# zhengchen1999/DOVE

Measured on AMD Instinct MI355X. Metric: SR frames/s (33x720x1280 4x one-step, whole job), higher is better.
Workload: dtype bf16; 1 GPU; synthetic 33x720x1280 HR clip (LR 180x320, 4x), one-step t=399, CogVideoX1.5-5B VAE + 42-layer DiT random-init, 1 clip per GPU (BASELINE configs[1]); weight_sums=True, vae_streams=2, variant=headline (bf16)

## Files before the change

### dove_amd/csrc/igemm.hip

```cpp
#include "igemm_args.h"


template <int BN, int BK>
struct FastCfg {
  static constexpr int BM = 128;
  static constexpr int CPR = BK / 8;
  static constexpr int CPR_LOG = (BK == 64) ? 3 : 2;
  static constexpr int RPG = 256 / CPR;
  static constexpr int NA = BM / RPG;
  static constexpr int B_SLOTS = BN * CPR;
  static constexpr int NB = (B_SLOTS + 255) / 256;
  static constexpr int A_BYTES = BM * BK * 2, B_BYTES = BN * BK * 2, STAGE = A_BYTES + B_BYTES;
  static constexpr int WN = (BN >= 128) ? 2 : 1, WM = 4 / WN;
  static constexpr int PT = (BM / WM) / 32, CT = (BN / WN) / 32;
  static constexpr int KK = BK / 16;
};

template <int BN, int BK>
__global__ __launch_bounds__(256) void igemm_fast_kernel(const IgemmArgs a) {
  using Cf = FastCfg<BN, BK>;
  constexpr int NA = Cf::NA, NB = Cf::NB, PT = Cf::PT, CT = Cf::CT, KK = Cf::KK, STAGE = Cf::STAGE, A_BYTES = Cf::A_BYTES;
  extern __shared__ __attribute__((aligned(16))) char smem[];
  const int tid = threadIdx.x, lane = tid & 63;
  const int wave = __builtin_amdgcn_readfirstlane(tid >> 6);
// ... 546 lines not shown
      mfma16(32 + 2 * g, wh[(2 * g) >> 3], xs[SP][(2 * g) & 7]);
      mfma16(32 + 2 * g + 1, wh[(2 * g + 1) >> 3], xs[SP][(2 * g + 1) & 7]);
      if (g < 8) {
        int ad;
        if (tap < NT - 1) ad = a16_addr(std::integral_constant<int, (tap + 1) % NT>{}, Par{}, g);
        else if (kSub) ad = a16_addr_next0(NPar{}, g);
        else ad = a16_addr(I0{}, NPar{}, g);
        xs[SP ^ 1][g] = *(const bf16x8*)(smem + ad);
      } else if (g < 12) {
        wl[g - 8] = *(const bf16x8*)(smem + b16_addr(SlotNxt{}, g - 8));
      }
      __builtin_amdgcn_sched_barrier(0);
    }
  };
  auto group = [&](auto parc) {
    step(std::integral_constant<int, 0>{}, parc); step(std::integral_constant<int, 1>{}, parc);
    step(std::integral_constant<int, 2>{}, parc); step(std::integral_constant<int, 3>{}, parc);
    if (!kSub) {
      step(std::integral_constant<int, (kSub ? 0 : 4)>{}, parc); step(std::integral_constant<int, (kSub ? 0 : 5)>{}, parc);
      step(std::integral_constant<int, (kSub ? 0 : 6)>{}, parc); step(std::integral_constant<int, (kSub ? 0 : 7)>{}, parc);
      step(std::integral_constant<int, (kSub ? 0 : 8)>{}, parc);
    }
  };

  const int e_px = lane >> 3, e_ch = lane & 7;
  for (int tile = (int)blockIdx.x; tile < ntiles; tile += G) {
    const H4Tile c = h4_decode<kPart>(a, kc, tile);
    f32x4 bias_r[2][2];
#pragma unroll
    for (int h = 0; h < 2; ++h) {
      const int cbh = c.n0 + h * 64 + e_ch * 8;
      bias_r[h][0] = bias_r[h][1] = f32x4{0.f, 0.f, 0.f, 0.f};
      if (a.bias) { bias_r[h][0] = *(const f32x4*)(a.bias + cbh); bias_r[h][1] = *(const f32x4*)(a.bias + cbh + 4); }
    }
#pragma unroll
    for (int k = 0; k < 64; ++k) acc16[k] = f32x4{0.f, 0.f, 0.f, 0.f};

    const int ng_tile = h4_split_ndt(a, __builtin_amdgcn_readfirstlane(h4_split(a, c.t))) * kc.kcn;
    int next_base0 = 0;
    if (kSub) {
      sub_bases(c.ph, abaseT);
      int nb4[4];
      sub_bases(h4_decode(a, kc, tile + G).ph, nb4);
      next_base0 = nb4[0];
    }
#pragma unroll
    for (int idx = 0; idx < 8; ++idx) xs[0][idx] = *(const bf16x8*)(smem + a16_addr(I0{}, I0{}, idx));
#pragma unroll
    for (int ib = 0; ib < 4; ++ib) wl[ib] = *(const bf16x8*)(smem + b16_addr(I0{}, ib));
    for (int g = 0; g < ng_tile; g += 2) {
      if (kSub) abaseN0 = abaseT[0];
      group(I0{});
      __builtin_amdgcn_sched_barrier(0);
      h4_advance<kUp, kPart>(st, a, kc);
      publish(st);
      __builtin_amdgcn_sched_barrier(0);
      if (kSub) abaseN0 = (g + 2 >= ng_tile) ? next_base0 : abaseT[0];
      group(I1{});
      __builtin_amdgcn_sched_barrier(0);
      h4_advance<kUp, kPart>(st, a, kc);
      publish(st);
      __builtin_amdgcn_sched_barrier(0);
    }

    __builtin_amdgcn_s_barrier();
    {
      constexpr int EROW = 272;
      char* const eslice = smem + A_BYTES + wave * 12288;
      unsigned o_off[4], r_off[4];
#pragma unroll
      for (int it = 0; it < 4; ++it) {
        const int px = it * 8 + e_px;
        if (kPart == 1) {
          const int col = px & 15, row = px >> 4;
          const bool okw = c.ow0 + col < a.w_lim;
          o_off[it] = okw ? (unsigned)(((row * a.W_out + col) * (int)a.ldo + e_ch * 8) * 2) : 0x80000000u;
          r_off[it] = okw ? (unsigned)(((row * a.W_out + col) * (int)a.ldr + e_ch * 8) * 2) : 0x80000000u;
          continue;
        }
        const bool okw = kSub ? c.ow0 + px < a.W_in : c.ow0 + px < a.w_lim;
        o_off[it] = okw ? (unsigned)(((kSub ? 2 * px : px) * (int)a.ldo + e_ch * 8) * 2) : 0x80000000u;
        r_off[it] = okw ? (unsigned)((px * (int)a.ldr + e_ch * 8) * 2) : 0x80000000u;
      }
      auto emit = [&](auto has_resid, auto has_gn) {
        constexpr bool kRes = decltype(has_resid)::value;
        constexpr bool kGn = decltype(has_gn)::value;
        typedef __attribute__((ext_vector_type(2))) float f32x2;
        f32x2 gs[2][2], gq[2][2];
#pragma unroll
        for (int h = 0; h < 2; ++h)
#pragma unroll
          for (int q2 = 0; q2 < 2; ++q2) { gs[h][q2] = f32x2{0.f, 0.f}; gq[h][q2] = f32x2{0.f, 0.f}; }
        auto wr = [&](int p, int h) {
#pragma unroll
          for (int ib = 0; ib < 4; ++ib)
#pragma unroll
            for (int j = 0; j < 2; ++j) *(f32x4*)(eslice + (16 * j + l15) * EROW + (ib * 16 + 4 * q4) * 4) = acc16[(h * 4 + ib) * 8 + 2 * p + j];
          (void)hi; (void)l31;
        };
        auto gn_flush = [&](int half) {
          const int cpg_log = a.cpg_log;
          const int gty = (c.oh0 >> 4) + (kPart == 1 ? wave >> 1 : 0), gtx = c.ow0 >> 5;
          const int slot = kPart == 1 ? 2 * (wave & 1) + half : wave;
          const long long tix = ((long long)c.t * a.tiles_h + gty) * a.tiles_w + gtx;
          const long long row = ((kSub ? tix * 4 + c.ph : tix) << 2) + slot;
          float* dst = a.gn_partial + row * 64;
          const bool own = kPart != 1 || (gty < a.tiles_h && gty * 16 < a.h_lim);
#pragma unroll
          for (int h = 0; h < 2; ++h) {
            float sv[2], qv[2];
#pragma unroll
            for (int q2 = 0; q2 < 2; ++q2) {
              sv[q2] = gs[h][q2][0] + gs[h][q2][1];
              qv[q2] = gq[h][q2][0] + gq[h][q2][1];
#pragma unroll
              for (int m = 8; m < 64; m <<= 1) { sv[q2] += __shfl_xor(sv[q2], m); qv[q2] += __shfl_xor(qv[q2], m); }
              gs[h][q2] = f32x2{0.f, 0.f}; gq[h][q2] = f32x2{0.f, 0.f};
            }
            const int ch0 = c.n0 + h * 64 + e_ch * 8;
            if (cpg_log == 2) {
              if (e_px == 0 && own) {
                dst[(ch0 >> 2) * 2] = sv[0]; dst[(ch0 >> 2) * 2 + 1] = qv[0];
                dst[((ch0 >> 2) + 1) * 2] = sv[1]; dst[((ch0 >> 2) + 1) * 2 + 1] = qv[1];
              }
            } else {
              float s8 = sv[0] + sv[1], q8 = qv[0] + qv[1];
              if (cpg_log == 4) { s8 += __shfl_xor(s8, 1); q8 += __shfl_xor(q8, 1); }
              const bool writer = e_px == 0 && (cpg_log == 3 || (e_ch & 1) == 0);
              if (writer && own) { dst[(ch0 >> cpg_log) * 2] = s8; dst[(ch0 >> cpg_log) * 2 + 1] = q8; }
            }
          }
        };
        wr(0, 0);
#pragma unroll
        for (int p = 0; p < 4; ++p) {
          const int oh = c.oh0 + RPW * wave + (kPart == 1 ? 2 * p : p);
          const long long pix0 = kSub ? ((long long)c.t * a.H_out + 2 * oh + (c.ph >> 1)) * a.W_out + 2 * c.ow0 + (c.ph & 1)
                                      : ((long long)c.t * a.H_out + oh) * a.W_out + c.ow0;
          const bool okh = kSub ? oh < a.H_in : oh < a.h_lim;
          const int span_px = kSub ? 2 * halo8::TW : (kPart == 1 ? a.W_out + 16 : halo8::TW);
          const auto srd_o = __builtin_amdgcn_make_buffer_rsrc((void*)(a.out + pix0 * a.ldo + c.n0), (short)0,
                                                               okh ? (int)(span_px * a.ldo * 2) : 0, 0x00020000);
          const auto srd_r = __builtin_amdgcn_make_buffer_rsrc((void*)(kRes ? a.resid + pix0 * a.ldr + c.n0 : a.out), (short)0,
                                                               (kRes && okh) ? (int)((kPart == 1 ? a.W_out + 16 : halo8::TW) * a.ldr * 2) : 0, 0x00020000);
          unsigned oo[4], ro[4];
          const bool ok1 = oh + 1 < a.h_lim;
#pragma unroll
          for (int it = 0; it < 4; ++it) {
            if (kPart == 1) { oo[it] = (it >= 2 && !ok1) ? 0x80000000u : o_off[it]; ro[it] = (it >= 2 && !ok1) ? 0x80000000u : r_off[it]; }
            else { oo[it] = o_off[it]; ro[it] = r_off[it]; }
          }
#pragma unroll
          for (int h = 0; h < 2; ++h) {
            u32x4 rr[4];
            if (kRes) {
#pragma unroll
              for (int it = 0; it < 4; ++it) rr[it] = __builtin_amdgcn_raw_buffer_load_b128(srd_r, (int)ro[it], h * 128, 0);
            }
            asm volatile("s_waitcnt lgkmcnt(0)" ::: "memory");
            f32x4 lo[4], hi4[4];
#pragma unroll
            for (int it = 0; it < 4; ++it) {
              lo[it] = *(const f32x4*)(eslice + (it * 8 + e_px) * EROW + e_ch * 32);
              hi4[it] = *(const f32x4*)(eslice + (it * 8 + e_px) * EROW + e_ch * 32 + 16);
            }
            asm volatile("s_waitcnt lgkmcnt(0)" ::: "memory");
            if (p < 3 || h < 1) wr(h ? p + 1 : p, h ^ 1);
#pragma unroll
            for (int it = 0; it < 4; ++it) {
              f32x4 x0 = lo[it] + bias_r[h][0], x1 = hi4[it] + bias_r[h][1];
              if (kRes) {
                const u32x4 r = rr[it];
                x0 += f32x4{__uint_as_float(r[0] << 16), __uint_as_float(r[0] & 0xffff0000u), __uint_as_float(r[1] << 16),
                            __uint_as_float(r[1] & 0xffff0000u)};
                x1 += f32x4{__uint_as_float(r[2] << 16), __uint_as_float(r[2] & 0xffff0000u), __uint_as_float(r[3] << 16),
                            __uint_as_float(r[3] & 0xffff0000u)};
              }
              const u32x4 v = {pack_bf2(x0[0], x0[1]), pack_bf2(x0[2], x0[3]), pack_bf2(x1[0], x1[1]), pack_bf2(x1[2], x1[3])};
              if (kGn) {
                const bool valid = okh && oo[it] != 0x80000000u;
#pragma unroll
                for (int e = 0; e < 4; ++e) {
                  const uint32_t w = valid ? v[e] : 0u;
                  const f32x2 f = {__uint_as_float(w << 16), __uint_as_float(w & 0xffff0000u)};
                  gs[h][e >> 1] += f;
                  gq[h][e >> 1] += f * f;
                }
              }
              __builtin_amdgcn_raw_buffer_store_b128(v, srd_o, (int)oo[it], h * 128, 0);
              __builtin_amdgcn_sched_barrier(0);
              asm volatile("s_nop 3" ::: "memory");
              __builtin_amdgcn_sched_barrier(0);
            }
          }
          if (kGn && kPart == 1 && p == 1) gn_flush(0);
        }
        if (kGn) gn_flush(kPart == 1 ? 1 : 0);
      };
      if (a.gn_partial) {
        if (a.resid) emit(std::true_type{}, std::true_type{});
        else emit(std::false_type{}, std::true_type{});
      } else {
        if (a.resid) emit(std::true_type{}, std::false_type{});
        else emit(std::false_type{}, std::false_type{});
      }
    }
    asm volatile("s_waitcnt vmcnt(0)" ::: "memory");
  }
}

namespace gemm8p {
constexpr int ROWB = 128;
constexpr int OPB = 256 * ROWB;
constexpr int XB = 0, WB = 2 * OPB;
constexpr int EPI = 4 * OPB;
constexpr int LDS_BYTES = EPI + 8 * 4096;
}
template <bool kAct, bool kGate>
__global__ __launch_bounds__(512, 2) void gemm8p_kernel(const IgemmArgs a, long long M) {
  using gemm4x::BM;
  using namespace gemm8p;
  extern __shared__ __attribute__((aligned(16))) char smem[];
  const int tid = threadIdx.x, lane = tid & 63;
  const int wave = __builtin_amdgcn_readfirstlane(tid >> 6);
  __builtin_assume(wave >= 0 && wave < 8);
  const int hi = lane >> 5, l31 = lane & 31;
  const int q4 = lane >> 4, l15 = lane & 15;
  const int grp = wave >> 2, wc = wave & 3;

  G4Const kc;
  kc.K = a.Cin;
  kc.M = M;
  kc.tiles_n = a.tiles_n;
  kc.ntiles = (int)((M + BM - 1) / BM) * a.tiles_n;
  kc.G = (int)gridDim.x;
  kc.nk4 = a.Cin / 128;
  const int ntiles = kc.ntiles, G = kc.G, nk4 = kc.nk4;

  unsigned voff[4];
#pragma unroll
  for (int jj = 0; jj < 4; ++jj) {
    const int row = (wave * 4 + jj) * 8 + (lane >> 3);
    const int c = (lane & 7) ^ ((row >> 1) & 7);
    voff[jj] = (unsigned)((row * a.Cin + c * 8) * 2);
  }
  G4State st;
  const bf16_t *ca_base = a.x, *cw_base = a.w, *na_base = a.x, *nw_base = a.w;
  int ca_nrec = 0, cw_nrec = 0, c_soff = 0, na_nrec = 0, nw_nrec = 0, n_soff = 0;
  auto publish = [&](const G4State& q) {
    ca_base = na_base; cw_base = nw_base; ca_nrec = na_nrec; cw_nrec = nw_nrec; c_soff = n_soff;
    na_base = q.a_base; nw_base = q.w_base; na_nrec = q.a_nrec; nw_nrec = q.w_nrec; n_soff = q.soff;
  };
  auto stage = [&](auto bufc, const bf16_t* ab, int anrec, const bf16_t* wb, int wnrec, int soff) {
    constexpr int buf = decltype(bufc)::value;
    const auto srd_a = __builtin_amdgcn_make_buffer_rsrc((void*)ab, (short)0, anrec, 0x00020000);
    const auto srd_w = __builtin_amdgcn_make_buffer_rsrc((void*)wb, (short)0, wnrec, 0x00020000);
#pragma unroll
    for (int jj = 0; jj < 4; ++jj)
      __builtin_amdgcn_raw_ptr_buffer_load_lds(srd_a, (lds_ptr_t)(smem + XB + buf * OPB + wave * 4096 + jj * 1024), 16, voff[jj], soff, 0, 0);
#pragma unroll
    for (int jj = 0; jj < 4; ++jj)
      __builtin_amdgcn_raw_ptr_buffer_load_lds(srd_w, (lds_ptr_t)(smem + WB + buf * OPB + wave * 4096 + jj * 1024), 16, voff[jj], soff, 0, 0);
  };

  int aoff[2][2], boff[2][2];
  {
    const int ra = grp * 128 + l31, rb = wc * 64 + l31;
#pragma unroll
    for (int h = 0; h < 2; ++h)
#pragma unroll
      for (int kk = 0; kk < 2; ++kk) {
        const int ch = h * 4 + kk * 2 + hi;
        aoff[h][kk] = XB + ra * ROWB + ((ch ^ ((ra >> 1) & 7)) << 4);
        boff[h][kk] = WB + rb * ROWB + ((ch ^ ((rb >> 1) & 7)) << 4);
        asm volatile("" : "+v"(aoff[h][kk]), "+v"(boff[h][kk]));
// ... 265 lines not shown
                          d->t_in == d->t_out && d->h_in == d->h_out && d->w_in == d->w_out && d->cout_pad % 128 == 0 && M >= 4096 &&
                          (long long)512 * d->cin * 2 < (1ll << 31);
  const bool pointwise = d->kt == 1 && d->kh == 1 && d->kw == 1 && d->stride == 1 && d->up == 0 && d->tmode == 0 && d->t_in == d->t_out &&
                         d->h_in == d->h_out && d->w_in == d->w_out;
  if (pointwise && d->cin == 32 && d->act == 0 && !d->resid && !d->gate && d->cout_store >= 128) return K_SMALLK;
  if (plain_gemm) {
    if (d->cout_pad % 256 == 0 && d->cout_store % 256 == 0 && d->cin % 128 == 0 && d->cin >= 256 && (long long)256 * d->cin * 2 < (1ll << 31) &&
        d->ldo < (1 << 20) && d->ldr < (1 << 20) && (d->act == 0 || d->act == 1))
      return K_GEMM8P;
  }
  const bool conv3 = d->kh == 3 && d->kw == 3 && d->stride == 1 && d->pad_h == 1 && d->pad_w == 1 && d->act == 0 && !d->gate &&
                     d->cout_pad % 128 == 0 && frame_fits;
  if (conv3) {
    const bool same = d->up == 0 && d->tmode == 0 && d->h_out == d->h_in && d->w_out == d->w_in && d->w_out >= 16 && d->h_out >= 16;
    const bool ups = d->up == 1 && d->kt == 1 && d->h_out == 2 * d->h_in && d->w_out == 2 * d->w_in && d->h_out >= 16 && d->w_out >= 32;
    const bool h4 = d->cout_store % 128 == 0 && d->cin % 64 == 0 && d->ldo < (1 << 20) && (!d->resid || d->ldr < (1 << 20));
    if (same && h4) return K_HALO4X;
    if (ups && h4 && d->w_sub && d->h_in >= 16 && d->w_in >= 32) return K_HALO4X_SUB;
    if (ups && h4) return K_HALO4X_UP;
  }
  const int BN = (d->cout_pad % 128 == 0) ? 128 : ((d->cout_pad % 64 == 0) ? 64 : 32);
  const bool fits = frame_fits && (long long)BN * d->cin * 2 < (1ll << 31);
  return (d->up == 0 && fits) ? K_IGEMM_FAST : K_IGEMM;
}

static bool desc_size_ok(const dove_conv_desc* d, const char* who) {
  if (d && d->struct_size == sizeof(dove_conv_desc) && d->reserved == 0) return true;
  if (d) dove_set_error("%s: dove_conv_desc.struct_size is %u, this library (ABI %d) expects %zu - the caller's binding was written "
                        "against another include/dove_hip.h", who, d->struct_size, DOVE_ABI_VERSION, sizeof(dove_conv_desc));
  else dove_set_error("%s: null descriptor", who);
  return false;
}
extern "C" const char* dove_conv_kernel_name(const dove_conv_desc* d) { return desc_size_ok(d, "conv_kernel_name") ? kKernelNames[select_kernel(d)] : ""; }

template <int BN, int BK>
static int launch_igemm_fast(const IgemmArgs& a, unsigned grid, hipStream_t s) {
  constexpr int lds = 2 * (128 * BK * 2 + BN * BK * 2);
  static PerDeviceOnce attr_set;
  if (auto once_ = attr_set.guard()) (void)hipFuncSetAttribute((const void*)igemm_fast_kernel<BN, BK>, hipFuncAttributeMaxDynamicSharedMemorySize, lds);
  hipLaunchKernelGGL((igemm_fast_kernel<BN, BK>), dim3(grid), dim3(256), lds, s, a);
  DOVE_CHECK_LAUNCH("dove_conv_igemm_bf16");
  return DOVE_OK;
}

static int cu_count() {
  static std::atomic<int> cus[DOVE_MAX_DEVICES] = {};
  int dev = 0;
  (void)hipGetDevice(&dev);
  int n = (dev >= 0 && dev < DOVE_MAX_DEVICES) ? cus[dev].load(std::memory_order_relaxed) : 0;
  if (!n) {
    n = 256;
    (void)hipDeviceGetAttribute(&n, hipDeviceAttributeMultiprocessorCount, dev);
    if (dev >= 0 && dev < DOVE_MAX_DEVICES) cus[dev].store(n, std::memory_order_relaxed);
  }
  return n;
}

extern "C" long long dove_conv_gn_partial_rows(const dove_conv_desc* d) {
  if (!desc_size_ok(d, "conv_gn_partial_rows")) return 0;
  const ConvKernel k = select_kernel(d);
  if (k != K_HALO4X && k != K_HALO4X_UP && k != K_HALO4X_SUB) return 0;
  if (d->cout_store != 128 && d->cout_store != 256 && d->cout_store != 512) return 0;
  if (d->cout_store != d->cout_pad) return 0;
  if (k == K_HALO4X_SUB) {
    const long long th = (d->h_in + halo8::TH - 1) / halo8::TH, tw = (d->w_in + halo8::TW - 1) / halo8::TW;
    return (long long)desc_nb(d) * d->t_out * th * tw * 16;
  }
  const long long th = (d->h_out + halo8::TH - 1) / halo8::TH, tw = (d->w_out + halo8::TW - 1) / halo8::TW;
  return (long long)desc_nb(d) * d->t_out * th * tw * 4;
}

static bool halo4x_plan(const dove_conv_desc* d) {
  const int tiles_w = (d->w_out + halo8::TW - 1) / halo8::TW, tiles_h = (d->h_out + halo8::TH - 1) / halo8::TH;
  const int wrem = d->w_out % halo8::TW;
  if (wrem < 1 || wrem > halo8::TW / 2) return false;
  const int cus = cu_count();
  const long long per = (long long)desc_nb(d) * d->t_out * (d->cout_pad / 128);
  auto rounds = [&](long long tiles) { return (tiles * per + cus - 1) / cus; };
  return rounds((long long)tiles_h * (tiles_w - 1)) + rounds((d->h_out + 31) / 32) < rounds((long long)tiles_h * tiles_w);
}
extern "C" int dove_conv_partial_launches(const dove_conv_desc* d) {
  if (!desc_size_ok(d, "conv_partial_launches") || select_kernel(d) != K_HALO4X) return 0;
  return halo4x_plan(d) ? 1 : 0;
}

static int conv_dispatch(const dove_conv_desc* d, void* stream, ConvKernel kern);

static bool gemm_tail_split(const dove_conv_desc* d, long long* rows_main) {
  const long long M = (long long)d->t_out * d->h_out * d->w_out;
  if (d->t_out != 1 || d->h_out != 1 || desc_nb(d) > 1) return false;
  const int cus = cu_count(), tiles_n = d->cout_pad / 256;
  const long long row_tiles = (M + gemm4x::BM - 1) / gemm4x::BM, ntiles = row_tiles * tiles_n;
  if (ntiles <= cus || ntiles % cus == 0) return false;
  const long long main_rt = (ntiles / cus) * cus / tiles_n;
  if (main_rt < 1 || main_rt >= row_tiles) return false;
  const long long tail_rows = M - main_rt * gemm4x::BM;
  const long long tail_blocks = ((tail_rows + 127) / 128) * (d->cout_pad / 128);
  if (tail_blocks > 2ll * cus) return false;
  if ((long long)128 * d->cin * 2 >= (1ll << 31)) return false;
  *rows_main = main_rt * gemm4x::BM;
  return true;
}

extern "C" int dove_conv_igemm_bf16(const dove_conv_desc* d, void* stream) {
  if (!desc_size_ok(d, "conv_igemm")) return DOVE_EINVAL;
  DOVE_CHECK_ARG(d->x && d->w && d->out, "conv_igemm: null pointer");
  DOVE_CHECK_ARG(d->cin % 32 == 0 && d->cin > 0, "conv_igemm: Cin (%d) must be a positive multiple of 32 (pad on pack)", d->cin);
  DOVE_CHECK_ARG(d->cout_pad % 32 == 0 && d->cout_pad > 0, "conv_igemm: Cout_pad (%d) must be a multiple of 32", d->cout_pad);
  DOVE_CHECK_ARG(d->cout_store % 4 == 0 && d->cout_store <= d->cout_pad && d->cout_store > 0, "conv_igemm: bad cout_store %d", d->cout_store);
  DOVE_CHECK_ARG(d->ldo % 4 == 0 && d->ldo >= d->cout_store, "conv_igemm: ldo (%lld) must be a multiple of 4 and >= cout_store", d->ldo);
  DOVE_CHECK_ARG(!d->resid || (d->ldr % 4 == 0 && d->ldr >= d->cout_store), "conv_igemm: bad ldr %lld", d->ldr);
  DOVE_CHECK_ARG(!d->gate || d->resid, "conv_igemm: gate needs resid");
  DOVE_CHECK_ARG(d->kt >= 1 && d->kt <= 3 && d->kh >= 1 && d->kw >= 1, "conv_igemm: bad kernel size");
  DOVE_CHECK_ARG(d->stride == 1 || d->stride == 2, "conv_igemm: stride must be 1 or 2");
  DOVE_CHECK_ARG(d->up == 0 || d->up == 1, "conv_igemm: up must be 0/1");
  DOVE_CHECK_ARG(d->kt == 1 || (d->tmode == 0 && d->t_in == d->t_out), "conv_igemm: causal temporal taps need t_in == t_out and tmode 0");
  DOVE_CHECK_ARG(d->t_out > 0 && d->h_out > 0 && d->w_out > 0 && d->t_in > 0 && d->h_in > 0 && d->w_in > 0, "conv_igemm: empty tensor");
  DOVE_CHECK_ARG(d->nb >= 0 && d->nb <= 4096 && (long long)desc_nb(d) * d->t_out < (1 << 20), "conv_igemm: bad instance count nb = %d", d->nb);
  DOVE_CHECK_ARG(d->cache_stride == 0 || (d->cache && d->cache_stride >= (long long)(d->kt - 1) * d->h_in * d->w_in * d->cin),
                 "conv_igemm: cache_stride (%lld) is smaller than one instance's cache", d->cache_stride);
  DOVE_CHECK_ARG(desc_nb(d) == 1 || !d->gate, "conv_igemm: nb > 1 is not combined with gate");
  DOVE_CHECK_ARG(d->reserved2 == 0 && d->tdup >= 0 && d->tdup <= 2, "conv_igemm: bad tdup %d", d->tdup);
  DOVE_CHECK_ARG(!d->tdup || (d->kt == 3 && d->w_pair), "conv_igemm: tdup declares frame pairs of a kt == 3 conv and needs w_pair");
  DOVE_CHECK_ARG(!d->tdup || d->cache || d->w_first, "conv_igemm: tdup without a conv cache needs w_first too (frames whose three taps read one frame)");
  DOVE_CHECK_ARG(d->tdup != 2 || !d->cache, "conv_igemm: tdup == 2 (first frame single) is the head of a clip: no conv cache");
  DOVE_CHECK_ARG(!d->gn_partial || dove_conv_gn_partial_rows(d) > 0,
                 "conv_igemm: gn_partial requested but this call does not dispatch to a kernel that fuses the statistics");
  const ConvKernel kern0 = select_kernel(d);
  DOVE_CHECK_ARG(!d->out_f32 || (kern0 == K_IGEMM_FAST && !d->resid && d->act == 0),
                 "conv_igemm: out_f32 is only implemented for plain convs that dispatch to igemm_fast_kernel");
  long long rows_main = 0;
  if (kern0 == K_GEMM8P && gemm_tail_split(d, &rows_main)) {
    dove_conv_desc m = *d, t = *d;
    m.w_in = m.w_out = (int)rows_main;
    const long long tail = (long long)d->w_out - rows_main;
    t.w_in = t.w_out = (int)tail;
    t.x = (const char*)d->x + rows_main * d->cin * 2;
    t.out = (char*)d->out + rows_main * d->ldo * 2;
    if (d->resid) t.resid = (const char*)d->resid + rows_main * d->ldr * 2;
    t.gate_split = d->gate_split > rows_main ? d->gate_split - rows_main : 0;
    const int rc = conv_dispatch(&m, stream, K_GEMM8P);
    return rc ? rc : conv_dispatch(&t, stream, K_IGEMM_FAST);
  }
  return conv_dispatch(d, stream, kern0);
}

static int conv_dispatch(const dove_conv_desc* d, void* stream, ConvKernel kern) {
  const bf16_t* zp = zero_page();
  DOVE_CHECK_ARG(zp, "conv_igemm: could not allocate the zero page");
  IgemmArgs a;
  a.x = (const bf16_t*)d->x; a.cache = (const bf16_t*)d->cache; a.w = (const bf16_t*)d->w;
  a.bias = d->bias; a.resid = (const bf16_t*)d->resid; a.gate = d->gate; a.out = (bf16_t*)d->out; a.zero = zp;
  const int nb = desc_nb(d);
  a.T_out = nb * d->t_out; a.H_out = d->h_out; a.W_out = d->w_out;
  a.T_in = nb * d->t_in; a.H_in = d->h_in; a.W_in = d->w_in;
  a.seg_out = d->t_out; a.seg_in = d->t_in;
  a.cache_bs = d->cache_stride ? d->cache_stride : (long long)(d->kt - 1) * d->h_in * d->w_in * d->cin;
  a.Cin = d->cin; a.Cout_pad = d->cout_pad; a.Cout_st = d->cout_store;
  a.kt = d->kt; a.kh = d->kh; a.kw = d->kw; a.stride = d->stride; a.pad_h = d->pad_h; a.pad_w = d->pad_w;
  a.up = d->up; a.tmode = d->tmode; a.act = d->act; a.ldo = d->ldo; a.ldr = d->ldr; a.gate_split = d->gate_split;
  a.gn_partial = nullptr; a.cpg_log = 0;
  a.w_first = nullptr;
  a.w_pair = nullptr; a.tdup = 0;
  a.sub = 0;
  a.out_f32 = d->out_f32;
  a.nt_out = 0;
  a.reserved = 0;
  hipStream_t s = (hipStream_t)stream;
  const long long M = (long long)nb * d->t_out * d->h_out * d->w_out;
  switch (kern) {
    case K_GEMM8P: {
      a.tiles_n = d->cout_pad / 256;
      a.nt_out = (long long)M * d->ldo * 2 > (256ll << 20);
      const long long nt = ((M + gemm4x::BM - 1) / gemm4x::BM) * a.tiles_n;
      DOVE_CHECK_ARG(nt > 0 && nt < (1ll << 31), "conv_igemm: grid too large");
      DOVE_CHECK_ARG(!(d->gate && d->act), "conv_igemm: gate with activation is not a path of the reference");
      const int cus = cu_count();
      const unsigned grid4 = nt > cus ? (unsigned)cus : (unsigned)nt;
      static PerDeviceOnce attr8;
      if (auto once_ = attr8.guard()) {
        (void)hipFuncSetAttribute((const void*)gemm8p_kernel<false, false>, hipFuncAttributeMaxDynamicSharedMemorySize, gemm8p::LDS_BYTES);
        (void)hipFuncSetAttribute((const void*)gemm8p_kernel<true, false>, hipFuncAttributeMaxDynamicSharedMemorySize, gemm8p::LDS_BYTES);
        (void)hipFuncSetAttribute((const void*)gemm8p_kernel<false, true>, hipFuncAttributeMaxDynamicSharedMemorySize, gemm8p::LDS_BYTES);
      }
      if (d->gate) hipLaunchKernelGGL((gemm8p_kernel<false, true>), dim3(grid4), dim3(512), gemm8p::LDS_BYTES, s, a, M);
      else if (d->act == 1) hipLaunchKernelGGL((gemm8p_kernel<true, false>), dim3(grid4), dim3(512), gemm8p::LDS_BYTES, s, a, M);
      else hipLaunchKernelGGL((gemm8p_kernel<false, false>), dim3(grid4), dim3(512), gemm8p::LDS_BYTES, s, a, M);
      DOVE_CHECK_LAUNCH("dove_conv_igemm_bf16(gemm8p)");
      return DOVE_OK;
    }
    case K_SMALLK: {
      dim3 grid((unsigned)((M + 4 * smallk::ROWS - 1) / (4 * smallk::ROWS)), (unsigned)((d->cout_store + 255) / 256));
      hipLaunchKernelGGL(smallk_kernel, grid, dim3(256), 0, s, a.x, a.w, a.bias, a.out, M, d->cout_store, d->ldo);
      DOVE_CHECK_LAUNCH("dove_conv_igemm_bf16(smallk)");
      return DOVE_OK;
    }
    case K_HALO4X_SUB: {
      a.gn_partial = d->gn_partial;
      a.cpg_log = d->cout_store == 128 ? 2 : (d->cout_store == 256 ? 3 : 4);
      a.sub = 1;
      a.w = (const bf16_t*)d->w_sub;
      a.ty0 = a.tx0 = 0;
      a.tiles_w = (d->w_in + halo8::TW - 1) / halo8::TW;
      a.tiles_h = (d->h_in + halo8::TH - 1) / halo8::TH;
      a.tiles_n = 4 * (d->cout_pad / 128);
      a.nty = a.tiles_h; a.ntx = a.tiles_w; a.h_lim = d->h_out; a.w_lim = d->w_out;
      const long long g4 = (long long)a.T_out * a.tiles_h * a.tiles_w * a.tiles_n;
      DOVE_CHECK_ARG(g4 > 0 && g4 < (1ll << 31), "conv_igemm: grid too large");
      static PerDeviceOnce attrs;
      if (auto once_ = attrs.guard()) (void)hipFuncSetAttribute((const void*)(conv3x3_halo4x_kernel<false, true>), hipFuncAttributeMaxDynamicSharedMemorySize, Halo4xCfg::LDS_BYTES);
      const int cus = cu_count();
      const unsigned grid = g4 > cus ? (unsigned)cus : (unsigned)g4;
      hipLaunchKernelGGL((conv3x3_halo4x_kernel<false, true>), dim3(grid), dim3(256), Halo4xCfg::LDS_BYTES, s, a);
      DOVE_CHECK_LAUNCH("dove_conv_igemm_bf16(halo4x sub-pixel)");
      return DOVE_OK;
    }
    case K_HALO4X:
    case K_HALO4X_UP: {
      a.gn_partial = d->gn_partial;
      a.w_first = (kern == K_HALO4X && d->kt == 3 && !d->cache) ? (const bf16_t*)d->w_first : nullptr;
      if (kern == K_HALO4X && d->kt == 3 && d->tdup) { a.tdup = d->tdup; a.w_pair = (const bf16_t*)d->w_pair; }
      a.cpg_log = d->cout_store == 128 ? 2 : (d->cout_store == 256 ? 3 : 4);
      a.tiles_w = (d->w_out + halo8::TW - 1) / halo8::TW;
      a.tiles_h = (d->h_out + halo8::TH - 1) / halo8::TH;
      a.tiles_n = d->cout_pad / 128;
      a.ty0 = a.tx0 = 0; a.nty = a.tiles_h; a.ntx = a.tiles_w; a.h_lim = d->h_out; a.w_lim = d->w_out;
      const long long g4 = (long long)a.T_out * a.tiles_h * a.tiles_w * a.tiles_n;
      DOVE_CHECK_ARG(g4 > 0 && g4 < (1ll << 31), "conv_igemm: grid too large");
      static PerDeviceOnce attr4;
      if (auto once_ = attr4.guard()) {
        (void)hipFuncSetAttribute((const void*)(conv3x3_halo4x_kernel<false>), hipFuncAttributeMaxDynamicSharedMemorySize, Halo4xCfg::LDS_BYTES);
        (void)hipFuncSetAttribute((const void*)(conv3x3_halo4x_kernel<false, false, 1>), hipFuncAttributeMaxDynamicSharedMemorySize, H4Geo<1>::LDS_BYTES);
        (void)hipFuncSetAttribute((const void*)(conv3x3_halo4x_kernel<true>), hipFuncAttributeMaxDynamicSharedMemorySize, Halo4xCfg::LDS_BYTES);
      }
      const int cus = cu_count();
      const unsigned grid = g4 > cus ? (unsigned)cus : (unsigned)g4;
      if (kern == K_HALO4X_UP) hipLaunchKernelGGL((conv3x3_halo4x_kernel<true>), dim3(grid), dim3(256), Halo4xCfg::LDS_BYTES, s, a);
      else {
        const bool wpart = halo4x_plan(d);
        const int wm = wpart ? (a.tiles_w - 1) * halo8::TW : d->w_out, cols_main = wpart ? a.tiles_w - 1 : a.tiles_w;
        auto launch = [&](int part, int nty, int tx0, int ntx, int w_lim) {
          if (nty <= 0 || ntx <= 0) return;
          IgemmArgs b = a;
          b.ty0 = 0; b.nty = nty; b.tx0 = tx0; b.ntx = ntx; b.h_lim = d->h_out; b.w_lim = w_lim;
          const long long g = (long long)b.T_out * nty * ntx * b.tiles_n;
          const unsigned gr = g > cus ? (unsigned)cus : (unsigned)g;
          if (part == 0) hipLaunchKernelGGL((conv3x3_halo4x_kernel<false, false, 0>), dim3(gr), dim3(256), H4Geo<0>::LDS_BYTES, s, b);
          else hipLaunchKernelGGL((conv3x3_halo4x_kernel<false, false, 1>), dim3(gr), dim3(256), H4Geo<1>::LDS_BYTES, s, b);
        };
        launch(0, a.tiles_h, 0, cols_main, wm);
        if (wpart) launch(1, (d->h_out + 31) / 32, cols_main, 1, d->w_out);
      }
      DOVE_CHECK_LAUNCH("dove_conv_igemm_bf16(halo4x)");
      return DOVE_OK;
    }
    default: break;
  }
  int twl = 7;
  if (d->h_out > 1) {
    twl = 4;
    if (d->w_out <= 8) twl = 3;
    if (d->w_out <= 4) twl = 2;
  }
  a.tw_log2 = twl;
  const int TW = 1 << twl, TH = 128 >> twl;
  a.tiles_w = (d->w_out + TW - 1) / TW;
  a.tiles_h = (d->h_out + TH - 1) / TH;
  const int BN = (d->cout_pad % 128 == 0) ? 128 : ((d->cout_pad % 64 == 0) ? 64 : 32);
  a.tiles_n = d->cout_pad / BN;
  const long long grid = (long long)a.T_out * a.tiles_h * a.tiles_w * a.tiles_n;
  DOVE_CHECK_ARG(grid > 0 && grid < (1ll << 31), "conv_igemm: grid too large");
  const bool fast = kern == K_IGEMM_FAST;
  const bool bk64 = (d->cin % 64 == 0);
  if (!fast) return launch_igemm_legacy(a, (unsigned)grid, BN, bk64, s);
  if (BN == 128) return bk64 ? launch_igemm_fast<128, 64>(a, (unsigned)grid, s) : launch_igemm_fast<128, 32>(a, (unsigned)grid, s);
  if (BN == 64) return bk64 ? launch_igemm_fast<64, 64>(a, (unsigned)grid, s) : launch_igemm_fast<64, 32>(a, (unsigned)grid, s);
  return bk64 ? launch_igemm_fast<32, 64>(a, (unsigned)grid, s) : launch_igemm_fast<32, 32>(a, (unsigned)grid, s);
}
```

### dove_amd/csrc/igemm_args.h

```cpp
#pragma once
#include <stdlib.h>

#include <type_traits>

#include "common.h"
#include "../../include/dove_hip.h"

struct IgemmArgs {
  const bf16_t* x;
  const bf16_t* cache;
  const bf16_t* w;
  const float* bias;
  const bf16_t* resid;
  const float* gate;
  bf16_t* out;
  const bf16_t* zero;
  int T_out, H_out, W_out;
  int T_in, H_in, W_in;
  int Cin, Cout_pad, Cout_st;
  int kt, kh, kw, stride, pad_h, pad_w, up, tmode, act;
  long long ldo, ldr;
  long long gate_split;
  int tw_log2, tiles_w, tiles_h, tiles_n;
  int reserved;
  float* gn_partial;
  int cpg_log;
  int out_f32;
  int nt_out;
  int seg_out, seg_in;
  long long cache_bs;
  const bf16_t* w_first;
  const bf16_t* w_pair;
  int tdup;
  int ty0, tx0, nty, ntx;
  int h_lim, w_lim;
  int sub;
};

__device__ __forceinline__ const bf16_t* igemm_src_frame(const IgemmArgs& a, int t, int dt, long long frame_elems) {
  const int b = a.seg_out == a.T_out ? 0 : t / a.seg_out;
  const int tl = t - b * a.seg_out;
  const long long f0 = (long long)b * a.seg_in;
  if (a.kt > 1) {
    const int fv = tl + dt - (a.kt - 1);
    if (fv >= 0) return a.x + (f0 + fv) * frame_elems;
    if (a.cache) return a.cache + (long long)b * a.cache_bs + (long long)(a.kt - 1 + fv) * frame_elems;
    return a.x + f0 * frame_elems;
  }
  const int tin = a.tmode == 0 ? tl : (a.tmode == 1 ? (tl >> 1) : (tl == 0 ? 0 : 1 + ((tl - 1) >> 1)));
  return a.x + (f0 + tin) * frame_elems;
}

typedef __attribute__((address_space(3))) void* lds_ptr_t;

namespace gemm4x {
constexpr int BM = 256, BN = 256;
constexpr int ROWB = 64;
}
struct G4Tile { int m0, n0; };
struct G4Const { int ntiles, G, tiles_n, nk4, K; long long M; };
struct G4State {
  int n_tile, n_k4;
  bool n_on;
  const bf16_t *a_base, *w_base;
  int a_nrec, w_nrec, soff;
};
__device__ __forceinline__ G4Tile g4_decode(const G4Const& k, int id) {
  const unsigned rest = xcd_remap((unsigned)(id < k.ntiles ? id : k.ntiles - 1), (unsigned)k.ntiles);
  const unsigned GM = k.tiles_n > 16 ? 8u : 1u;
  const unsigned tiles_m = (unsigned)(k.ntiles / k.tiles_n);
  const unsigned per_group = GM * (unsigned)k.tiles_n;
  const unsigned group = rest / per_group, within = rest - group * per_group;
  const unsigned left = tiles_m - group * GM;
  const unsigned gm = left < GM ? left : GM;
  G4Tile q;
  q.m0 = __builtin_amdgcn_readfirstlane((int)(group * GM + within % gm) * gemm4x::BM);
  q.n0 = __builtin_amdgcn_readfirstlane((int)(within / gm) * gemm4x::BN);
  return q;
}
__device__ __forceinline__ void g4_open_tile(G4State& s, const IgemmArgs& a, const G4Const& k, int id) {
  s.n_tile = id;
  s.n_on = id < k.ntiles;
  const G4Tile q = g4_decode(k, id);
  const long long left = k.M - q.m0;
  const int rows = left < gemm4x::BM ? (int)left : gemm4x::BM;
  s.a_base = a.x + (long long)q.m0 * k.K;
  s.w_base = a.w + (long long)q.n0 * k.K;
  s.a_nrec = s.n_on ? rows * k.K * 2 : 0;
  s.w_nrec = s.n_on ? gemm4x::BN * k.K * 2 : 0;
  s.n_k4 = 0;
  s.soff = 0;
}
__device__ __forceinline__ void g4_advance(G4State& s, const IgemmArgs& a, const G4Const& k) {
  if (++s.n_k4 == k.nk4) g4_open_tile(s, a, k, s.n_tile + k.G);
  s.soff = s.n_k4 * (4 * gemm4x::ROWB);
}

int launch_igemm_legacy(const IgemmArgs& a, unsigned grid, int BN, bool bk64, hipStream_t s);
```

### dove_amd/ops.py

```python
from __future__ import annotations

import ctypes as C
import math
from dataclasses import dataclass

import numpy as np
import torch

from . import lib as L


def _ru(x: int, m: int) -> int:
    return (x + m - 1) // m * m


@dataclass
class PackedConv:
    w: torch.Tensor
    bias: torch.Tensor | None
    kt: int
    kh: int
    kw: int
    cin: int
    cin_pad: int
# ... 99 lines not shown
    return L.load().dove_conv_kernel_name(C.byref(d)).decode()


def conv(x: torch.Tensor, pc: PackedConv, *, cache: torch.Tensor | None = None, stride: int = 1, pad=(None, None),
         up: int = 0, tmode: int = 0, t_out: int | None = None, hw_out=None, resid: torch.Tensor | None = None,
         gate: torch.Tensor | None = None, gate_split: int = 0, act: int = 0, ldo: int | None = None,
         out: torch.Tensor | None = None,
         gn_eps: float | None = None, out_f32: bool = False, nb: int = 1, tdup: int = 0, weight_sums: bool = True) -> torch.Tensor:
    L.require_cuda(x, resid, gate, out)
    assert x.dtype == torch.bfloat16 and x.dim() == 4, (x.dtype, x.shape)
    T, H, W, Cx = x.shape
    assert T % nb == 0, (T, nb)
    T //= nb
    if Cx != pc.cin_pad:
        raise RuntimeError(f"conv: input has {Cx} channels, packed weight expects {pc.cin_pad}")
    ph = (pc.kh - 1) // 2 if pad[0] is None else pad[0]
    pw = (pc.kw - 1) // 2 if pad[1] is None else pad[1]
    if t_out is None:
        t_out = T
    if hw_out is None:
        hw_out = (H << up, W << up) if stride == 1 else ((H + 1 - pc.kh) // stride + 1, (W + 1 - pc.kw) // stride + 1)
    if ldo is None:
        ldo = pc.cout_store
    odt = torch.float32 if out_f32 else torch.bfloat16
    if out is None:
        out = torch.empty(nb * t_out, hw_out[0], hw_out[1], ldo, dtype=odt, device=x.device)
    else:
        assert out.shape == (nb * t_out, hw_out[0], hw_out[1], ldo) and out.dtype == odt
    cache_stride = 0
    if cache is not None:
        if nb > 1:
            assert cache.shape == (nb, pc.kt - 1, H, W, Cx) and cache.dtype == torch.bfloat16 and cache.is_cuda, (cache.shape, x.shape)
            assert cache[0].is_contiguous() and cache.device == x.device
            cache_stride = cache.stride(0)
        else:
            L.require_cuda(cache)
            assert cache.shape == (pc.kt - 1, H, W, Cx) and cache.dtype == torch.bfloat16, (cache.shape, x.shape)
    d = L.ConvDesc()
    d.nb, d.cache_stride = nb, cache_stride
    if cache is None and pc.w_first is not None and weight_sums:
        d.w_first = pc.w_first.data_ptr()
    if up == 1 and pc.w_sub is not None and weight_sums:
        d.w_sub = pc.w_sub.data_ptr()
    if tdup and weight_sums and pc.w_pair is not None and pc.kt == 3 and not (tdup == 2 and cache is not None):
        d.tdup, d.w_pair = tdup, pc.w_pair.data_ptr()
    d.x, d.cache, d.w = x.data_ptr(), (cache.data_ptr() if cache is not None else None), pc.w.data_ptr()
    d.bias = pc.bias.data_ptr() if pc.bias is not None else None
    d.resid = resid.data_ptr() if resid is not None else None
    d.gate = gate.data_ptr() if gate is not None else None
    d.out = out.data_ptr()
    d.t_in, d.h_in, d.w_in, d.cin = T, H, W, Cx
    d.t_out, d.h_out, d.w_out = t_out, hw_out[0], hw_out[1]
    d.cout_pad, d.cout_store = pc.cout_pad, pc.cout_store
    d.kt, d.kh, d.kw, d.stride, d.pad_h, d.pad_w = pc.kt, pc.kh, pc.kw, stride, ph, pw
    d.up, d.tmode, d.act = up, tmode, act
    d.ldo = ldo
    d.ldr = resid.shape[-1] if resid is not None else 0
    d.gate_split = gate_split
    d.out_f32 = int(out_f32)
    if resid is not None:
        assert resid.dtype == torch.bfloat16 and resid.numel() == nb * t_out * hw_out[0] * hw_out[1] * resid.shape[-1]
    if gate is not None:
        assert gate.dtype == torch.float32 and gate.shape == (2, pc.cout_pad)
    partial = None
    if gn_eps is not None and ldo == pc.cout_store:
        rows = int(L.load().dove_conv_gn_partial_rows(C.byref(d)))
        if rows > 0:
            partial = torch.empty(rows, 64, dtype=torch.float32, device=x.device)
            d.gn_partial = partial.data_ptr()
    if _profiler is not None:
        e0, e1 = torch.cuda.Event(enable_timing=True), torch.cuda.Event(enable_timing=True)
        e0.record()
    L.check(L.load().dove_conv_igemm_bf16(C.byref(d), L.stream_ptr()), "dove_conv_igemm_bf16")
    if _profiler is not None:
        e1.record()
        flops = 2.0 * nb * t_out * hw_out[0] * hw_out[1] * pc.cout * pc.cin * pc.kt * pc.kh * pc.kw
        name = L.load().dove_conv_kernel_name(C.byref(d)).decode()
        real = flops
        if name == "conv3x3_halo4x_kernel":
            if d.tdup and pc.kt == 3 and up == 0:
                real = flops * sum(temporal_groups(tl, d.tdup, cache is not None) for tl in range(t_out)) / (3.0 * t_out)
            elif d.w_first and pc.kt == 3 and up == 0:
                real = flops * (1.0 - (2.0 + (1.0 if t_out > 1 else 0.0)) / (3.0 * t_out))
            elif d.w_sub and up == 1 and H >= 16 and W >= 32:
                real = flops * 4.0 / 9.0
        _profiler.append(((pc.cin, pc.cout, pc.kt * pc.kh * pc.kw), flops, e0, e1, name, real))
    if partial is None:
        if getattr(out, "gn_stats", None) is not None:
            out.gn_stats = None
            out.gn_rows = None
    else:
        count = float(t_out * hw_out[0] * hw_out[1]) * (pc.cout_store // 32)
        if nb > 1:
            stats = torch.empty(nb, 32, 2, dtype=torch.float32, device=x.device)
            ws = _ws(x.device, nb * 512)
            L.check(L.load().dove_groupnorm_finalize_partials_nb(partial.data_ptr(), partial.shape[0] // nb, nb, count, gn_eps, L.ptr(ws),
                                                                 ws.numel() * 4, L.ptr(stats), L.stream_ptr()), "dove_groupnorm_finalize_partials_nb")
        else:
            stats = torch.empty(32, 2, dtype=torch.float32, device=x.device)
            L.check(L.load().dove_groupnorm_finalize_partials(partial.data_ptr(), partial.shape[0], count, gn_eps, L.ptr(_ws(x.device)),
                                                              L.ptr(stats), L.stream_ptr()), "dove_groupnorm_finalize_partials")
        out.gn_stats = (stats, gn_eps, out._version)
        out.gn_rows = partial
    return out


def groupnorm_stats_of(x: torch.Tensor, eps: float, nb: int = 1) -> torch.Tensor:
    have = getattr(x, "gn_stats", None)
    if have is not None and have[1] == eps and have[2] == x._version and have[0].numel() == nb * 64:
        return have[0]
    return groupnorm_stats(x, eps, nb)


def linear(x: torch.Tensor, pc: PackedConv, **kw) -> torch.Tensor:
    N = x.shape[0]
    out = kw.pop("out", None)
    resid = kw.pop("resid", None)
    y = conv(x.view(1, 1, N, x.shape[1]), pc, resid=None if resid is None else resid.view(1, 1, N, resid.shape[1]),
             out=None if out is None else out.view(1, 1, N, out.shape[1]), **kw)
    return y.view(N, y.shape[-1])


_gn_ws: dict = {}
GN_WS_ROWS = 4096


def _ws(device, rows: int = GN_WS_ROWS):
    key = (str(device), torch.cuda.current_stream(device).cuda_stream if torch.cuda.is_available() else 0)
    rows = max(rows, GN_WS_ROWS)
    if key not in _gn_ws or _gn_ws[key].numel() < rows * 64:
        _gn_ws[key] = torch.empty(rows * 64, dtype=torch.float32, device=device)
    return _gn_ws[key]


def _gn_rows_needed(x, frames: int) -> int:
    fp = _frame_pix(x) or x.numel() // x.shape[-1]
    nsub = 256 // max(x.shape[-1] // 8, 1)
    return frames * min(256, -(-fp // (max(nsub, 1) * 32)))


def _frame_pix(x):
    return x.shape[1] * x.shape[2] if x.dim() == 4 else 0


def groupnorm_stats(x: torch.Tensor, eps: float, nb: int = 1) -> torch.Tensor:
    L.require_cuda(x)
    assert x.dtype == torch.bfloat16
    Cc = x.shape[-1]
    frames = x.shape[0] if x.dim() == 4 else 1
    ws = _ws(x.device, _gn_rows_needed(x, frames))
    if nb > 1:
        assert x.dim() == 4 and x.shape[0] % nb == 0
        stats = torch.empty(nb, 32, 2, dtype=torch.float32, device=x.device)
        L.check(L.load().dove_groupnorm_stats_nb_bf16(L.ptr(x), nb, x.numel() // Cc // nb, _frame_pix(x), Cc, eps, L.ptr(ws), ws.numel() // 64,
                                                      L.ptr(stats), L.stream_ptr()), "dove_groupnorm_stats_nb_bf16")
        return stats
    stats = torch.empty(32, 2, dtype=torch.float32, device=x.device)
    L.check(L.load().dove_groupnorm_stats_bf16(L.ptr(x), x.numel() // Cc, _frame_pix(x), Cc, eps, L.ptr(ws), ws.numel() // 64, L.ptr(stats),
                                               L.stream_ptr()), "dove_groupnorm_stats_bf16")
    return stats


def groupnorm_sums(x: torch.Tensor) -> torch.Tensor:
    L.require_cuda(x)
    assert x.dtype == torch.bfloat16
    Cc = x.shape[-1]
    sums = torch.empty(32, 2, dtype=torch.float64, device=x.device)
    ws = _ws(x.device, _gn_rows_needed(x, x.shape[0] if x.dim() == 4 else 1))
# ... 1570 lines not shown
```

Before: 35.91 frames/s.

## Compute temporally duplicated upsample conv frames once and store to both outputs

For 1x1-temporal upsampling convs whose temporal mode duplicates input frames (tmode 1/2, no residual), the halo4x kernels now iterate over source frames instead of output frames. Each computed tile is written to both duplicated output frames, and its GroupNorm partial statistics are written twice. This removes redundant conv compute on identical duplicated frames in the VAE decoder upsample path, at the cost of extra stores and slightly more index logic in the epilogue.

```diff
diff --git a/dove_amd/csrc/igemm.hip b/dove_amd/csrc/igemm.hip
--- a/dove_amd/csrc/igemm.hip
+++ b/dove_amd/csrc/igemm.hip
@@ -652,6 +652,16 @@
         o_off[it] = okw ? (unsigned)(((kSub ? 2 * px : px) * (int)a.ldo + e_ch * 8) * 2) : 0x80000000u;
         r_off[it] = okw ? (unsigned)((px * (int)a.ldr + e_ch * 8) * 2) : 0x80000000u;
       }
+      constexpr bool kPairs = kUp || kSub;
+      int ot = c.t;
+      bool two = false;
+      if (kPairs && a.tpair) {
+        const int b = a.seg_in == a.T_in ? 0 : c.t / a.seg_in;
+        const int sf = c.t - b * a.seg_in;
+        const int per = a.tpair == 1 ? 2 * a.seg_in : 2 * a.seg_in - 1;
+        ot = __builtin_amdgcn_readfirstlane(b * per + (a.tpair == 1 ? 2 * sf : (sf ? 2 * sf - 1 : 0)));
+        two = __builtin_amdgcn_readfirstlane((a.tpair == 1 || sf > 0) ? 1 : 0) != 0;
+      }
       auto emit = [&](auto has_resid, auto has_gn) {
         constexpr bool kRes = decltype(has_resid)::value;
         constexpr bool kGn = decltype(has_gn)::value;
@@ -672,10 +682,15 @@
           const int cpg_log = a.cpg_log;
           const int gty = (c.oh0 >> 4) + (kPart == 1 ? wave >> 1 : 0), gtx = c.ow0 >> 5;
           const int slot = kPart == 1 ? 2 * (wave & 1) + half : wave;
-          const long long tix = ((long long)c.t * a.tiles_h + gty) * a.tiles_w + gtx;
+          const long long tix = ((long long)ot * a.tiles_h + gty) * a.tiles_w + gtx;
           const long long row = ((kSub ? tix * 4 + c.ph : tix) << 2) + slot;
           float* dst = a.gn_partial + row * 64;
+          const long long dst2 = (long long)a.tiles_h * a.tiles_w * (kSub ? 16 : 4) * 64;
           const bool own = kPart != 1 || (gty < a.tiles_h && gty * 16 < a.h_lim);
+          auto put = [&](int g, float sum, float sq) {
+            dst[g * 2] = sum; dst[g * 2 + 1] = sq;
+            if (kPairs && two) { dst[dst2 + g * 2] = sum; dst[dst2 + g * 2 + 1] = sq; }
+          };
 #pragma unroll
           for (int h = 0; h < 2; ++h) {
             float sv[2], qv[2];
@@ -690,14 +705,14 @@
             const int ch0 = c.n0 + h * 64 + e_ch * 8;
             if (cpg_log == 2) {
               if (e_px == 0 && own) {
-                dst[(ch0 >> 2) * 2] = sv[0]; dst[(ch0 >> 2) * 2 + 1] = qv[0];
-                dst[((ch0 >> 2) + 1) * 2] = sv[1]; dst[((ch0 >> 2) + 1) * 2 + 1] = qv[1];
+                put(ch0 >> 2, sv[0], qv[0]);
+                put((ch0 >> 2) + 1, sv[1], qv[1]);
               }
             } else {
               float s8 = sv[0] + sv[1], q8 = qv[0] + qv[1];
               if (cpg_log == 4) { s8 += __shfl_xor(s8, 1); q8 += __shfl_xor(q8, 1); }
               const bool writer = e_px == 0 && (cpg_log == 3 || (e_ch & 1) == 0);
-              if (writer && own) { dst[(ch0 >> cpg_log) * 2] = s8; dst[(ch0 >> cpg_log) * 2 + 1] = q8; }
+              if (writer && own) put(ch0 >> cpg_log, s8, q8);
             }
           }
         };
@@ -705,12 +720,14 @@
 #pragma unroll
         for (int p = 0; p < 4; ++p) {
           const int oh = c.oh0 + RPW * wave + (kPart == 1 ? 2 * p : p);
-          const long long pix0 = kSub ? ((long long)c.t * a.H_out + 2 * oh + (c.ph >> 1)) * a.W_out + 2 * c.ow0 + (c.ph & 1)
-                                      : ((long long)c.t * a.H_out + oh) * a.W_out + c.ow0;
+          const long long pix0 = kSub ? ((long long)ot * a.H_out + 2 * oh + (c.ph >> 1)) * a.W_out + 2 * c.ow0 + (c.ph & 1)
+                                      : ((long long)ot * a.H_out + oh) * a.W_out + c.ow0;
           const bool okh = kSub ? oh < a.H_in : oh < a.h_lim;
           const int span_px = kSub ? 2 * halo8::TW : (kPart == 1 ? a.W_out + 16 : halo8::TW);
           const auto srd_o = __builtin_amdgcn_make_buffer_rsrc((void*)(a.out + pix0 * a.ldo + c.n0), (short)0,
                                                                okh ? (int)(span_px * a.ldo * 2) : 0, 0x00020000);
+          const auto srd_o2 = __builtin_amdgcn_make_buffer_rsrc((void*)(a.out + (pix0 + (kPairs ? (long long)a.H_out * a.W_out : 0)) * a.ldo + c.n0), (short)0,
+                                                                (kPairs && two && okh) ? (int)(span_px * a.ldo * 2) : 0, 0x00020000);
           const auto srd_r = __builtin_amdgcn_make_buffer_rsrc((void*)(kRes ? a.resid + pix0 * a.ldr + c.n0 : a.out), (short)0,
                                                                (kRes && okh) ? (int)((kPart == 1 ? a.W_out + 16 : halo8::TW) * a.ldr * 2) : 0, 0x00020000);
           unsigned oo[4], ro[4];
@@ -761,6 +778,12 @@
               __builtin_amdgcn_sched_barrier(0);
               asm volatile("s_nop 3" ::: "memory");
               __builtin_amdgcn_sched_barrier(0);
+              if (kPairs && two) {
+                __builtin_amdgcn_raw_buffer_store_b128(v, srd_o2, (int)oo[it], h * 128, 0);
+                __builtin_amdgcn_sched_barrier(0);
+                asm volatile("s_nop 3" ::: "memory");
+                __builtin_amdgcn_sched_barrier(0);
+              }
             }
           }
           if (kGn && kPart == 1 && p == 1) gn_flush(0);
@@ -1192,6 +1215,15 @@
 extern "C" int dove_conv_partial_launches(const dove_conv_desc* d) {
   if (!desc_size_ok(d, "conv_partial_launches") || select_kernel(d) != K_HALO4X) return 0;
   return halo4x_plan(d) ? 1 : 0;
+}
+
+static bool halo4x_pairs(const dove_conv_desc* d) {
+  return d->kt == 1 && d->up == 1 && (d->tmode == 1 || d->tmode == 2) && !d->resid &&
+         d->t_out == (d->tmode == 1 ? 2 * d->t_in : 2 * d->t_in - 1);
+}
+static void halo4x_walk_sources(IgemmArgs& a) {
+  a.tpair = a.tmode; a.tmode = 0;
+  a.T_out = a.T_in; a.seg_out = a.seg_in;
 }
 
 static int conv_dispatch(const dove_conv_desc* d, void* stream, ConvKernel kern);
@@ -1273,9 +1305,9 @@
   a.w_first = nullptr;
   a.w_pair = nullptr; a.tdup = 0;
   a.sub = 0;
+  a.tpair = 0;
   a.out_f32 = d->out_f32;
   a.nt_out = 0;
-  a.reserved = 0;
   hipStream_t s = (hipStream_t)stream;
   const long long M = (long long)nb * d->t_out * d->h_out * d->w_out;
   switch (kern) {
@@ -1315,6 +1347,7 @@
       a.tiles_h = (d->h_in + halo8::TH - 1) / halo8::TH;
       a.tiles_n = 4 * (d->cout_pad / 128);
       a.nty = a.tiles_h; a.ntx = a.tiles_w; a.h_lim = d->h_out; a.w_lim = d->w_out;
+      if (halo4x_pairs(d)) halo4x_walk_sources(a);
       const long long g4 = (long long)a.T_out * a.tiles_h * a.tiles_w * a.tiles_n;
       DOVE_CHECK_ARG(g4 > 0 && g4 < (1ll << 31), "conv_igemm: grid too large");
       static PerDeviceOnce attrs;
@@ -1335,6 +1368,7 @@
       a.tiles_h = (d->h_out + halo8::TH - 1) / halo8::TH;
       a.tiles_n = d->cout_pad / 128;
       a.ty0 = a.tx0 = 0; a.nty = a.tiles_h; a.ntx = a.tiles_w; a.h_lim = d->h_out; a.w_lim = d->w_out;
+      if (kern == K_HALO4X_UP && halo4x_pairs(d)) halo4x_walk_sources(a);
       const long long g4 = (long long)a.T_out * a.tiles_h * a.tiles_w * a.tiles_n;
       DOVE_CHECK_ARG(g4 > 0 && g4 < (1ll << 31), "conv_igemm: grid too large");
       static PerDeviceOnce attr4;
diff --git a/dove_amd/csrc/igemm_args.h b/dove_amd/csrc/igemm_args.h
--- a/dove_amd/csrc/igemm_args.h
+++ b/dove_amd/csrc/igemm_args.h
@@ -22,7 +22,7 @@
   long long ldo, ldr;
   long long gate_split;
   int tw_log2, tiles_w, tiles_h, tiles_n;
-  int reserved;
+  int tpair;
   float* gn_partial;
   int cpg_log;
   int out_f32;
diff --git a/dove_amd/ops.py b/dove_amd/ops.py
--- a/dove_amd/ops.py
+++ b/dove_amd/ops.py
@@ -205,8 +205,11 @@
                 real = flops * sum(temporal_groups(tl, d.tdup, cache is not None) for tl in range(t_out)) / (3.0 * t_out)
             elif d.w_first and pc.kt == 3 and up == 0:
                 real = flops * (1.0 - (2.0 + (1.0 if t_out > 1 else 0.0)) / (3.0 * t_out))
-            elif d.w_sub and up == 1 and H >= 16 and W >= 32:
-                real = flops * 4.0 / 9.0
+            elif up == 1:
+                if d.w_sub and H >= 16 and W >= 32:
+                    real = flops * 4.0 / 9.0
+                if pc.kt == 1 and tmode in (1, 2) and resid is None and t_out == (2 * T if tmode == 1 else 2 * T - 1):
+                    real = real * T / t_out
         _profiler.append(((pc.cin, pc.cout, pc.kt * pc.kh * pc.kw), flops, e0, e1, name, real))
     if partial is None:
         if getattr(out, "gn_stats", None) is not None:
```

Result: no change. 35.90 frames/s (-0.0%).
